# tuanad121/Python-WORLD

Measured on AMD Instinct MI355X. Metric: analysis+synthesis frames/sec (and xRT), 16 kHz / 5 ms hop, higher is better.
Workload: dtype f64; 1 GPU; BASELINE config 2 per GPU: 64 x 10 s synthetic 16 kHz utterances, DIO+StoneMask+CheapTrick+D4C encode + pulse-wise synthesis decode with on-device Philox noise (not the reference-parity host-noise path), HBM-resident; utterances_per_gpu=64, distinct_utterances=64, fs=16000, lanes_per_gpu=1

## Files before the change

### __graft_entry__.py

```python
import importlib.util
import os
import sys

ROOT = os.path.dirname(os.path.abspath(__file__))
PKG = os.path.join(ROOT, "python-world_amd")
for p in (ROOT, PKG):
    if p not in sys.path:
        sys.path.insert(0, p)


def build() -> None:
    spec = importlib.util.spec_from_file_location("_world_build", os.path.join(PKG, "build.py"))
    mod = importlib.util.module_from_spec(spec)
    spec.loader.exec_module(mod)
    lib = mod.build(force=False, verbose=True)
    assert os.path.exists(lib), lib
    from world import _hip

    handle = _hip.load_library()
    missing = [n for n in _hip.SIGNATURES if not hasattr(handle, n)]
    assert not missing, "missing C-ABI symbols: %s" % missing
    import oracle.api
    import subprocess

    from tests.test_hip_bounds import BOUNDS_TUS, VARIANT
    if not os.path.exists(VARIANT) or os.path.getmtime(VARIANT) < os.path.getmtime(lib):
        spec_arg = "bounds=" + ";".join("%s:-DWH_BOUNDS=1" % tu for tu in BOUNDS_TUS)
        r = subprocess.run([sys.executable, os.path.join(ROOT, "tools", "build_variants.py"), spec_arg], capture_output=True,
                           text=True)
        assert r.returncode == 0 and "bounds ok" in r.stdout, r.stdout[-2000:] + r.stderr[-2000:]
    from tests.test_hip_resample_bounds import VARIANT as RS_VARIANT, build_variant
    if not os.path.exists(RS_VARIANT) or os.path.getmtime(RS_VARIANT) < os.path.getmtime(lib):
        build_variant()
    from tests.test_hip_manifold_bounds import VARIANT as DS_VARIANT, build_variant as build_ds_variant
    if not os.path.exists(DS_VARIANT) or os.path.getmtime(DS_VARIANT) < os.path.getmtime(lib):
        build_ds_variant()
    from tests._fft_variant_script import VARIANT as NC_VARIANT, build_variant as build_nc_variant
    if not os.path.exists(NC_VARIANT) or os.path.getmtime(NC_VARIANT) < os.path.getmtime(lib):
        build_nc_variant()
    print("build ok:", lib, "ABI version", handle.wh_version(), "+ bounds variants")


def smoke() -> None:
    import numpy as np
    import torch

    assert torch.cuda.is_available(), "smoke() needs a GPU"
    from oracle import api as oapi
    from world._synthetic import synth_utterance
    from world.batch import WorldBatch

    fs = 16000
    xs = [synth_utterance(40, fs, 0.6), synth_utterance(41, fs, 0.5)]
    wb = WorldBatch(0)
    enc = wb.encode(xs, fs, f0_method="dio")
    rng = np.random.RandomState(0)
    noise = [rng.randn(2 * len(x)) for x in xs]
    y, y_off = wb.decode_device(enc, noise=noise)
    y = y.cpu().numpy()
    dicts = enc.to_dicts()
    for u, x in enumerate(xs):
        o = oapi.encode_np(fs, x, f0_method="dio")
        assert np.array_equal(dicts[u]["vuv"], o["vuv"])
        for key in ("f0", "spectrogram", "aperiodicity"):
            err = np.sqrt(np.mean((dicts[u][key] - o[key]) ** 2) / np.mean(o[key] ** 2))
            assert err < 1e-6, (key, err)
        yo = oapi.decode_np(dict(dicts[u]), noise=noise[u])["out"]
        seg = y[y_off[u]:y_off[u + 1]]
        assert len(seg) == len(yo)
        err = np.sqrt(np.mean((seg - yo) ** 2) / np.mean(yo ** 2))
        assert err < 1e-6, ("out", err)
    assert wb.rt.take_flags() == [0] * 16
    print("smoke ok: HIP encode+decode matches the oracle on %d utterances" % len(xs))


if __name__ == "__main__":
    build()
    if len(sys.argv) > 1 and sys.argv[1] == "smoke":
        smoke()
```

### python-world_amd/csrc/wh_synthesis.hip

```cpp
#include <type_traits>

#include "wh_host.h"
#include "wh_math.h"
__device__ __forceinline__ unsigned wh_opaque_tid() {
  unsigned t = threadIdx.x;
  asm volatile("" : "+v"(t));
  return t;
}
#define WH_TID wh_opaque_tid()
#include "wh_device.h"

#ifdef WH_RESP_STAGE_TIMER
__device__ unsigned long long g_resp_stage[16];
#define RSTAGE_BEGIN unsigned long long _t0 = __builtin_readcyclecounter();
#define RSTAGE_MARK(i) { __syncthreads(); if (threadIdx.x == 0) { const unsigned long long _t = __builtin_readcyclecounter(); atomicAdd(&g_resp_stage[i], _t - _t0); _t0 = _t; } }
#define RSTAGE_COUNT(i) { if (threadIdx.x == 0) atomicAdd(&g_resp_stage[i], 1ull); }
#else
#define RSTAGE_BEGIN
#define RSTAGE_MARK(i)
#define RSTAGE_COUNT(i)
#endif
namespace {

#ifndef WH_SYN_CONTRACT
#define WH_SYN_CONTRACT 0
#endif
#ifndef WH_RESP_TRANS_UNROLL
#define WH_RESP_TRANS_UNROLL 1
#endif
#ifndef WH_RESP_ABLATE
#define WH_RESP_ABLATE 0
#endif
#ifndef WH_RESP_ROLES
#define WH_RESP_ROLES 1
#endif
#ifndef WH_RESP_PAIR
#define WH_RESP_PAIR 1
#endif
#ifndef WH_RESP_SKIP_AP
#define WH_RESP_SKIP_AP 1
#endif
#ifndef WH_RESP_CONV8
#define WH_RESP_CONV8 1
#endif
#ifndef WH_FT_SYNTH
#define WH_FT_SYNTH 256
#endif
constexpr int ft_syn(int n) { return n >= 2048 ? 2 * WH_FT_SYNTH : WH_FT_SYNTH; }
template <int N>
constexpr bool resp_conv8() { return WH_RESP_CONV8 && N / ft_syn(N) == 4 && N >= 2048; }

struct SynUtt {
  int64_t f_off, nf;
  int64_t y_off, ny;
  int64_t p_off, pcap;
  int64_t noise_off, noise_len;
  double t0, dt;
};

__device__ __forceinline__ int64_t lerp_segment(const double* __restrict__ tp, int64_t nf, double t) {
  int64_t lo = 0, hi = nf;
  if (nf >= 2) {
    const double first = tp[0], last = tp[nf - 1];
    const double g = ceil((t - first) * (double)(nf - 1) / (last - first));
    if (g >= 1.0 && g <= (double)(nf - 1)) {
      const int64_t gi = (int64_t)g;
      const double a = tp[gi - 1], b = tp[gi], c = gi + 1 < nf ? tp[gi + 1] : b;
      if (a < t && !(b < t)) return gi;
      if (b < t && !(c < t) && gi + 1 <= nf - 1) return gi + 1;
      if (gi >= 2 && !(a < t) && tp[gi - 2] < t) return gi - 1;
    }
  }
  while (lo < hi) {
    const int64_t mid = (lo + hi) >> 1;
    if (tp[mid] < t) lo = mid + 1; else hi = mid;
  }
  return lo < 1 ? 1 : (lo > nf - 1 ? nf - 1 : lo);
}
__device__ __forceinline__ double lerp_on(const double* __restrict__ tp, const double* __restrict__ v, int64_t ih, double t) {
  const int64_t il = ih - 1;
  const double slope = (v[ih] - v[il]) / (tp[ih] - tp[il]);
  return slope * (t - tp[il]) + v[il];
}

__global__ __launch_bounds__(256) void prep_kernel(const SynUtt* __restrict__ meta, const double* __restrict__ tp,
                                                   const double* __restrict__ f0, const double* __restrict__ vuv,
                                                   double fs, double f0_low_limit, double* __restrict__ phase,
                                                   uint8_t* __restrict__ vuv_s) {
  const SynUtt m = meta[blockIdx.y];
  const int64_t i = (int64_t)blockIdx.x * 256 + threadIdx.x;
  if (i >= m.ny) return;
  const double t = m.t0 + (double)i * m.dt;
  const double* tpu = tp + m.f_off;
  const int64_t ih = lerp_segment(tpu, m.nf, t);
  double f_raw;
  if (f0_low_limit > 0.0) {
    const double* fu = f0 + m.f_off;
    const double* vu = vuv + m.f_off;
    auto final_f0 = [&](int64_t k) { return vu[k] == 0.0 ? 0.0 : (fu[k] < f0_low_limit ? 500.0 : fu[k]); };
    const int64_t il = ih - 1;
    const double slope = (final_f0(ih) - final_f0(il)) / (tpu[ih] - tpu[il]);
    f_raw = slope * (t - tpu[il]) + final_f0(il);
  } else {
    f_raw = lerp_on(tpu, f0 + m.f_off, ih, t);
  }
  const bool v = lerp_on(tpu, vuv + m.f_off, ih, t) > 0.5;
  double fi = f_raw * (v ? 1.0 : 0.0);
  if (fi == 0.0) fi = fi + 500.0;
  phase[m.y_off + i] = 2 * M_PI * fi / fs;
  vuv_s[m.y_off + i] = v ? 1 : 0;
}

#ifndef WH_XTILE
#define WH_XTILE 4096
#endif
constexpr int kXTile = WH_XTILE;
#ifndef WH_XTHREADS
#define WH_XTHREADS 512
#endif
constexpr int kXThreads = WH_XTHREADS;
// ... 604 lines not shown
  for (int r = 0; r < 10; ++r) {
    philox_round(c0, c1, c2, c3, k0, k1);
    k0 += 0x9E3779B9u;
    k1 += 0xBB67AE85u;
  }
  const double u1 = ((double)c0 * 4294967296.0 + (double)c1 + 0.5) * (1.0 / 18446744073709551616.0);
  const double u2 = ((double)c2 * 4294967296.0 + (double)c3 + 0.5) * (1.0 / 18446744073709551616.0);
  const double rr = sqrt(-2.0 * log(u1));
  double s, c;
  sincospi(2 * u2, &s, &c);
  return (q & 1) ? rr * s : rr * c;
}

__device__ __attribute__((noinline)) double2 normal_pair(uint64_t seed, uint64_t blk) {
  uint32_t c0 = (uint32_t)blk, c1 = (uint32_t)(blk >> 32), c2 = 0x9E3779B9u, c3 = 0x243F6A88u;
  uint32_t k0 = (uint32_t)seed, k1 = (uint32_t)(seed >> 32);
#pragma unroll
  for (int r = 0; r < 10; ++r) {
    philox_round(c0, c1, c2, c3, k0, k1);
    k0 += 0x9E3779B9u;
    k1 += 0xBB67AE85u;
  }
  const double u1 = ((double)c0 * 4294967296.0 + (double)c1 + 0.5) * (1.0 / 18446744073709551616.0);
  const double u2 = ((double)c2 * 4294967296.0 + (double)c3 + 0.5) * (1.0 / 18446744073709551616.0);
  const double rr = sqrt(-2.0 * log(u1));
  double s, c;
  sincospi(2 * u2, &s, &c);
  return make_double2(rr * c, rr * s);
}

__device__ __host__ __forceinline__ uint64_t philox_key(uint64_t seed, uint64_t u) {
  return seed * 0x9E3779B97F4A7C15ull + u * 0xD1B54A32D192ED03ull + 1;
}
__global__ __launch_bounds__(256) void philox_dump_kernel(uint64_t seed, int32_t u, int64_t q0, int64_t n,
                                                          double* __restrict__ out) {
  const int64_t i = (int64_t)blockIdx.x * 256 + threadIdx.x;
  if (i < n) out[i] = normal_at(philox_key(seed, (uint64_t)u), (uint64_t)(q0 + i));
}
__global__ __launch_bounds__(64) void noise_cover_kernel(const SynUtt* __restrict__ meta, const PulseRec* __restrict__ rec,
                                                         const int64_t* __restrict__ p_base, int n_utt,
                                                         int32_t* __restrict__ flags) {
  const int u = blockIdx.x * 64 + threadIdx.x;
  if (u >= n_utt) return;
  const int64_t count = p_base[u + 1] - p_base[u];
  if (count < 1) return;
  const PulseRec& r = rec[p_base[u] + count - 1];
  const int64_t need = r.noff + (r.noise_size > 3 ? r.noise_size : 3);
  if (meta[u].noise_len >= 0 && need > meta[u].noise_len) atomicOr(flags + WH_FLAG_NOISE_SHORT, 1);
}

#ifndef WH_FAST_MATH64
#define WH_FAST_MATH64 1
#endif
#ifndef WH_TRANS_PAIRS
#define WH_TRANS_PAIRS 1
#endif
__device__ __attribute__((noinline)) double4 cis_pair_call(double a0, double b0, double a1, double b1) {
  const double e0 = exp(a0), e1 = exp(a1);
  double s0, c0, s1, c1;
  sincospi(b0, &s0, &c0);
  sincospi(b1, &s1, &c1);
  return make_double4(e0 * c0, e0 * s0, e1 * c1, e1 * s1);
}
#if WH_FAST_MATH64
__device__ __attribute__((noinline)) double2 log_pair_call(double x, double y) { return make_double2(wh::flog(x), wh::flog(y)); }
__device__ __attribute__((noinline)) double log_call(double x) { return wh::flog(x); }
__device__ __attribute__((noinline)) double exp_call(double x) { return exp(x); }
__device__ __attribute__((noinline)) double2 sincospi_call(double x) {
  double s, c;
  sincospi(x, &s, &c);
  return make_double2(s, c);
}
#else
__device__ __attribute__((noinline)) double2 log_pair_call(double x, double y) { return make_double2(log(x), log(y)); }
__device__ __attribute__((noinline)) double log_call(double x) { return log(x); }
__device__ __attribute__((noinline)) double exp_call(double x) { return exp(x); }
__device__ __attribute__((noinline)) double2 sincospi_call(double x) {
  double s, c;
  sincospi(x, &s, &c);
  return make_double2(s, c);
}
#endif

template <int M, bool INV, int GT, int FT, bool WAVE>
__device__ __forceinline__ void mp_fft(wh::ckp<double2> zb, wh::ckp<const double2> tw) {
  if constexpr (WAVE) wh::fft_lds_wave<M, INV, GT, FT>(zb, tw);
  else wh::fft_lds<M, INV, GT, FT>(zb, tw);
}
template <int N>
constexpr bool resp_wave_fft() { return N == 1024; }
template <int N>
constexpr bool resp_skip_ap() { return WH_RESP_SKIP_AP && resp_wave_fft<N>(); }
struct SpectrumIdentity {
  __device__ __forceinline__ double2 operator()(int, double2 e) const { return e; }
};
struct NoSide {};
template <int N, int GT, bool WAVE = false, class Mul = SpectrumIdentity, class Side = NoSide>
__device__ __forceinline__ void min_phase_response(wh::ckp<double2> zb, wh::ckp<const double2> tw_base, double delay_pi, Mul mul = Mul(),
                                                   Side side = Side()) {
#if WH_SYN_CONTRACT
#pragma clang fp contract(fast)
#endif
  constexpr int FT = ft_syn(N);
  constexpr int M = N / 2;
  constexpr int PP = (M / 2 + 1 + GT - 1) / GT;
  const wh::ckp<double> zr = wh::ck_as<double>(zb);
  const int gt = WH_TID & (GT - 1);
  const wh::ckp<const double2> WH_RESTRICT w = tw_base + N;
#if defined(WH_RESP_ABLATE_T1) && WH_RESP_ABLATE_T1
  wh::sync<FT>();
#else
  if constexpr (WAVE && !std::is_same<Side, NoSide>::value) wh::fft_lds_wave<M, false, GT, FT>(zb, tw_base + M, side);
  else mp_fft<M, false, GT, FT, WAVE>(zb, tw_base + M);
#endif
  {
    double ck[PP], cm[PP];
#pragma unroll
    for (int p = 0; p < PP; ++p) {
      const int k = gt + p * GT;
      ck[p] = cm[p] = 0.0;
      if (k <= M / 2) {
        const double2 a = zb[k], b = zb[M - k];
        if (k == 0) {
          ck[p] = a.x + a.y;
          cm[p] = a.x - a.y;
        } else {
          const double er = 0.5 * (a.x + b.x), dr = 0.5 * (a.x - b.x), di = 0.5 * (a.y + b.y);
          const double2 wk = wh::ldg2(w + k);
          const double tr = fma(wk.x, di, wk.y * dr);
          ck[p] = er + tr;
          cm[p] = er - tr;
        }
      }
    }
    wh::sync<FT>();
#pragma unroll
    for (int p = 0; p < PP; ++p) {
      const int k = gt + p * GT;
      if (k <= M / 2) {
        if (k == 0) {
          zr[0] = ck[p];
          zr[M] = 2 * cm[p];
        } else {
          zr[N - k] = 2 * ck[p];
          zr[M + k] = 2 * cm[p];
        }
      }
    }
    for (int n = 1 + gt; n < M; n += GT) zr[n] = 0.0;
    wh::sync<FT>();
  }
  mp_fft<M, false, GT, FT, WAVE>(zb, tw_base + M);
#pragma unroll 1
  for (int k = gt; k <= M / 2; k += GT) {
    const double2 a = zb[k], b = zb[M - k];
    double2 x0, x1;
    const double2 wk = wh::ldg2(w + k);
    if (k == 0) {
      x0 = make_double2(a.x + a.y, 0.0);
      x1 = make_double2(a.x - a.y, 0.0);
    } else {
      const double er = 0.5 * (a.x + b.x), ei = 0.5 * (a.y - b.y);
      const double dr = 0.5 * (a.x - b.x), di = 0.5 * (a.y + b.y);
      const double tr = fma(wk.x, di, wk.y * dr);
      const double ti = fma(wk.y, di, -(wk.x * dr));
      x0 = make_double2(er + tr, ei + ti);
      x1 = make_double2(er - tr, ti - ei);
    }
#if WH_TRANS_PAIRS
    const double4 cis = cis_pair_call(x0.x / N, -x0.y / N * M_1_PI - delay_pi * (double)k, x1.x / N,
                                      -x1.y / N * M_1_PI - delay_pi * (double)(M - k));
    const double e0 = 1.0, e1 = 1.0;
    const double2 s0 = make_double2(cis.y, cis.x), s1 = make_double2(cis.w, cis.z);
#else
    const double e0 = exp_call(x0.x / N), e1 = exp_call(x1.x / N);
    const double2 s0 = sincospi_call(-x0.y / N * M_1_PI - delay_pi * (double)k);
    const double2 s1 = sincospi_call(-x1.y / N * M_1_PI - delay_pi * (double)(M - k));
#endif
    double2 A = mul(k, make_double2(e0 * s0.y, e0 * s0.x)), B = mul(M - k, make_double2(e1 * s1.y, e1 * s1.x));
    if (k == 0) {
      A.y = 0.0;
      B.y = 0.0;
    }
    const double er = A.x + B.x, ei = A.y - B.y;
    const double dr = A.x - B.x, di = A.y + B.y;
    const double orr = fma(dr, wk.x, di * wk.y);
    const double oi = fma(di, wk.x, -(dr * wk.y));
    zb[k] = make_double2(er - oi, ei + orr);
    if (k != 0) zb[M - k] = make_double2(er + oi, orr - ei);
  }
  wh::sync<FT>();
  mp_fft<M, true, GT, FT, WAVE>(zb, tw_base + M);
}

__device__ __forceinline__ int rap_index(int i) { return i + 2 * (i >> 5); }

__device__ __forceinline__ int first_pulse_at(const int64_t* __restrict__ pi, int count, int64_t lo) {
  const int lane = threadIdx.x & 63;
  int base = 0, n = count;
  while (n > 0) {
    const int stride = (n + 63) / 64;
    const int idx = base + lane * stride;
    const bool below = idx < base + n && pi[idx] < lo;
    const int c = __popcll(__ballot(below));
    if (stride == 1) {
      base += c;
      break;
    }
    if (c == 0) break;
    const int nb_ = base + (c - 1) * stride + 1;
    const int left = base + n - nb_;
    n = stride - 1 < left ? stride - 1 : left;
    base = nb_;
  }
  return base;
}

struct RespArgs {
  const SynUtt* meta;
  const double* tp;
  const double* spectrogram;
  const double* aperiodicity;
  double fs;
  const PulseRec* p_rec;
  const int64_t* p_base;
  int n_utt;
  const double* noise;
  uint64_t seed;
  const double* dc_base;
  const double2* tw_base;
  double* rows;
  const int64_t* row_base;
  const int64_t* run_base;
  const int64_t* row_off;
  int64_t runs_cap;
};

struct RunState {
  bool any;
  int64_t win_start;
  int64_t row_start;
  double last;
};
#ifndef WH_RESP_RUN
#define WH_RESP_RUN 0
#endif

template <int N>
__device__ __forceinline__ void ring_flush(wh::ckp<double> ring, int64_t a, int64_t b, wh::ckp<double> WH_RESTRICT row, int64_t row_start,
                                           int64_t ny) {
  constexpr int FT = ft_syn(N);
  a = a < 1 ? 1 : a;
  b = b > ny ? ny : b;
  for (int64_t tgt = a + WH_TID; tgt < b; tgt += FT) {
    const int slot = (int)(tgt & (N - 1));
    row[1 + (tgt - row_start)] = ring[slot];
    ring[slot] = 0.0;
  }
}

template <int R>
__device__ __forceinline__ void noise_conv_groups(wh::ckp<double> rap, wh::ckp<double> nzb, int cnt, int m0, int64_t j0, double (&acc)[R]) {
#if WH_SYN_CONTRACT
#pragma clang fp contract(fast)
#endif
  auto load_group = [&](int base, double (&g)[R]) {
#pragma unroll
    for (int t = 0; t < R; t += 2) {
      double2 v = make_double2(0.0, 0.0);
      if (base >= 0) v = wh::ck_as<const double2>(rap + rap_index(base + t))[0];
      g[t] = v.x;
      g[t + 1] = v.y;
    }
  };
  auto block = [&](int j, const double (&hi)[R], const double (&lo)[R]) {
    double n[R];
#pragma unroll
    for (int t = 0; t < R; t += 2) {
      const double2 v = wh::ck_as<const double2>(nzb + (j + t))[0];
      n[t] = v.x;
      n[t + 1] = v.y;
    }
#pragma unroll
    for (int sft = 0; sft < R; ++sft)
#pragma unroll
      for (int q = 0; q < R; ++q) acc[q] = fma(n[sft], q - sft >= 0 ? hi[q - sft] : lo[R + q - sft], acc[q]);
  };
  double ga[R], gb[R];
  const int mb0 = m0 - (int)j0;
  load_group(mb0, ga);
  load_group(mb0 - R, gb);
  const int steps = ((cnt + 2 * R - 1) / (2 * R)) * (2 * R);
  for (int j = 0; j < steps; j += 2 * R) {
    block(j, ga, gb);
    load_group(mb0 - j - 2 * R, ga);
    block(j + R, gb, ga);
    load_group(mb0 - j - 3 * R, gb);
  }
}

template <int N>
__device__ __forceinline__ void ring_advance(wh::ckp<double> ring, RunState& rs, wh::ckp<double> WH_RESTRICT row, int64_t s1, int64_t ny) {
  constexpr int FT = ft_syn(N);
  if (rs.any) {
    const int64_t e = s1 < rs.win_start + N ? s1 : rs.win_start + N;
    ring_flush<N>(ring, rs.win_start, e, row, rs.row_start, ny);
    for (int64_t tgt = rs.win_start + N + WH_TID; tgt < (s1 < ny ? s1 : ny); tgt += FT) row[1 + (tgt - rs.row_start)] = 0.0;
    wh::sync<FT>();
  } else {
    rs.row_start = s1 < 1 ? 1 : s1;
  }
  rs.any = true;
  rs.win_start = s1;
}

template <int N>
__device__ __forceinline__ void response_pulse(const RespArgs& A, const PulseRec& rec, char* smem, wh::ckp<double> ring, RunState& rs,
                                               wh::ckp<double> WH_RESTRICT row,
                                               const double (&dcw)[N / ft_syn(N) <= 4 ? N / ft_syn(N) : 1]) {
#if WH_SYN_CONTRACT
#pragma clang fp contract(fast)
#endif
  const SynUtt* __restrict__ meta = A.meta;
  const double* __restrict__ spectrogram = A.spectrogram;
  const double* __restrict__ aperiodicity = A.aperiodicity;
  const double fs = A.fs;
  const double* __restrict__ noise = A.noise;
  const uint64_t seed = A.seed;
  const double* __restrict__ dc_base = A.dc_base;
  const double2* __restrict__ tw_raw = A.tw_base;
  asm volatile("" : "+s"(tw_raw));
  const wh::ckp<const double2> tw_base = wh::ck_make(tw_raw, WH_TWIDDLE_ENTRIES, wh::WH_CK_TWIDDLE);
  constexpr int FT = ft_syn(N);
  constexpr int K = N / 2 + 1;
  constexpr int NZ = 256;
  constexpr int NZC = resp_conv8<N>() ? 252 : NZ;
  constexpr int R = N / FT;
  static_assert(R % 2 == 0 && NZ % (2 * R) == 0, "pairwise reads; whole blocks of 2R noise samples");
  constexpr int GT = FT >= 256 ? FT / 2 : FT;
  constexpr int NG = FT / GT;
  const wh::ckp<double> lds_all = wh::ck_make(reinterpret_cast<double*>(smem), 2 * (N + 2) + (N + N / 16 + 2) + NZ + 32, wh::WH_CK_LDS_OTHER);
  const wh::ckp<double> zrA = wh::ck_sub(lds_all, 0, N + 2, wh::WH_CK_LDS_MAIN);
  const wh::ckp<double2> zbA = wh::ck_as<double2>(zrA);
  const wh::ckp<double> zrP = wh::ck_sub(lds_all, N + 2, N + 2, wh::WH_CK_LDS_AUX);
  const wh::ckp<double2> zbP = wh::ck_as<double2>(zrP);
  const wh::ckp<double> rap = wh::ck_sub(lds_all, 2 * (N + 2), N + N / 16 + 2, wh::WH_CK_LDS_OTHER);
  const wh::ckp<double> nz = wh::ck_sub(lds_all, 2 * (N + 2) + (N + N / 16 + 2), NZ, wh::WH_CK_LDS_OTHER);
  const wh::ckp<double> scratch = wh::ck_sub(lds_all, 2 * (N + 2) + (N + N / 16 + 2) + NZ, 32, wh::WH_CK_LDS_SCRATCH);

  RSTAGE_BEGIN
  wh::sync<FT>();
  const int u = rec.u;
  const SynUtt m = meta[u];
  const int64_t pidx = rec.pidx;
  const double shift = rec.shift;
  const int64_t noise_size = rec.noise_size;

  const int64_t row_lo = rec.rows & 0xffffffffll, row_hi = rec.rows >> 32;
  const double bw = rec.weight;
  const bool same = bw < 0.0;
  const double b = same ? 0.0 : bw;
  const double a = 1 - b;
  const double* s_lo = spectrogram + row_lo * K;
  const double* s_hi = spectrogram + row_hi * K;
  const double* a_lo = aperiodicity + row_lo * K;
  const double* a_hi = aperiodicity + row_hi * K;
  constexpr int KQ = (K + FT - 1) / FT;
  double rsl[KQ], rsh[KQ], ral[KQ], rah[KQ];
  const bool need_ap = rec.vuv != 0;
#pragma unroll
  for (int q = 0; q < KQ; ++q) {
    const int k = WH_TID + q * FT;
    const int kc = k < K ? k : K - 1;
    rsl[q] = s_lo[kc];
    rsh[q] = s_hi[kc];
    if constexpr (resp_skip_ap<N>()) {
      ral[q] = rah[q] = 0.0;
    } else {
      ral[q] = a_lo[kc];
      rah[q] = a_hi[kc];
    }
  }
  double ap0_lo, ap0_hi;
  if constexpr (resp_skip_ap<N>()) {
    ap0_lo = ap0_hi = 0.0;
    if (need_ap) {
#pragma unroll
      for (int q = 0; q < KQ; ++q) {
        const int k = WH_TID + q * FT;
        const int kc = k < K ? k : K - 1;
        ral[q] = a_lo[kc];
        rah[q] = a_hi[kc];
      }
      ap0_lo = a_lo[0];
      ap0_hi = a_hi[0];
    }
  } else {
    ap0_lo = a_lo[0];
    ap0_hi = a_hi[0];
  }
  asm volatile("" : "+v"(ap0_lo), "+v"(ap0_hi));
  double aper0;
  {
    const double al = ap0_lo * ap0_lo, ah = ap0_hi * ap0_hi;
    aper0 = same ? al : a * al + b * ah;
  }
  const bool voiced = (rec.vuv != 0) && (aper0 <= 0.999);
  RSTAGE_COUNT(voiced ? 8 : (rec.vuv == 0 ? 9 : 10))
  RSTAGE_COUNT(13)
#pragma unroll
  for (int q = 0; q < KQ; ++q) {
    const int k = WH_TID + q * FT;
    if (k >= K) break;
    const double sl = rsl[q], sh = rsh[q];
    double v, w;
    auto spectra = [&]() {
      double al = ral[q] * ral[q], ah = rah[q] * rah[q];
      if constexpr (resp_skip_ap<N>()) asm volatile("" : "+v"(al), "+v"(ah));
      const double pl = fmax(0.001, 1 - al), ph = fmax(0.001, 1 - ah);
      const double sp = same ? sl : a * sl + b * sh;
      const double pe = same ? pl : a * pl + b * ph;
      const double ap = same ? al : a * al + b * ah;
      v = sp * pe;
      if (v == 0.0) v = 2.220446049250313e-16;
      w = voiced ? sp * ap : sp;
    };
    if constexpr (resp_skip_ap<N>()) {
      v = 0.0;
      w = same ? sl : a * sl + b * sh;
      if (voiced) spectra();
    } else {
      spectra();
    }
    if (w == 0.0) w = 2.220446049250313e-16;
#if WH_TRANS_PAIRS
    double2 lg;
    if (voiced) lg = log_pair_call(fabs(w), fabs(v));
    else lg = make_double2(log_call(fabs(w)), 0.0);
    const double lw = lg.x / 2;
#else
    const double lw = log_call(fabs(w)) / 2;
#endif
    zrA[k] = lw;
    if (k > 0 && k < N / 2) zrA[N - k] = lw;
    if (voiced) {
#if WH_TRANS_PAIRS
      const double lv = lg.y / 2;
#else
      const double lv = log_call(fabs(v)) / 2;
#endif
      zrP[k] = lv;
      if (k > 0 && k < N / 2) zrP[N - k] = lv;
    }
  }
  RSTAGE_MARK(5)
  const int64_t nd = noise_size > 3 ? noise_size : 3;
  const int64_t noff = rec.noff;
  auto noise_at = [&](int64_t j) -> double {
    if (noise) {
      const int64_t q = noff + j;
      return q < m.noise_len ? noise[m.noise_off + q] : 0.0;
    }
    return normal_at(philox_key(seed, (uint64_t)u), (uint64_t)(noff + j));
  };
  constexpr bool ROLES = WH_RESP_ROLES && resp_wave_fft<N>();
  static_assert(!ROLES || NZ / 2 + 1 <= FT, "a run that fits nz is at most one Philox block per thread");
  const bool side_noise = ROLES && noise == nullptr && nd <= NZ;
  auto noise_side = [&](int i, int n) {
    if (!side_noise) return;
    const uint64_t key = philox_key(seed, (uint64_t)u);
    const int lane = i & 63;
    const int64_t blk0 = noff >> 1, b1 = (noff + nd - 1) >> 1;
    for (int c = __builtin_amdgcn_readfirstlane(i - lane); blk0 + c <= b1; c += n) {
      const int64_t blk = blk0 + c + lane;
      double part = 0.0;
      if (blk <= b1) {
        const double2 z = normal_pair(key, (uint64_t)blk);
        const int64_t j = 2 * blk - noff;
        if (j >= 0) {
          part += z.x;
          nz[j] = z.x;
        }
        if (j + 1 < nd) {
          part += z.y;
          nz[j + 1] = z.y;
        }
      }
      part = wh::wave_sum(part);
      if (lane == 0) scratch[c >> 6] = part;
    }
  };
  double mean = 0.0;
  if (side_noise) {
    wh::sync<FT>();
  } else {
    double part = 0.0;
    if (noise) {
      for (int64_t j = WH_TID; j < nd; j += FT) {
        const double v = noise_at(j);
        part += v;
        if (j < NZ) nz[j] = v;
      }
    } else {
      const uint64_t key = philox_key(seed, (uint64_t)u);
      const int64_t b1 = (noff + nd - 1) >> 1;
      for (int64_t blk = (noff >> 1) + WH_TID; blk <= b1; blk += FT) {
        const double2 z = normal_pair(key, (uint64_t)blk);
        const int64_t j = 2 * blk - noff;
        if (j >= 0) {
          part += z.x;
          if (j < NZ) nz[j] = z.x;
        }
        if (j + 1 < nd) {
          part += z.y;
          if (j + 1 < NZ) nz[j + 1] = z.y;
        }
      }
    }
    mean = wh::block_sum<FT>(part, scratch) / (double)nd;
  }

  RSTAGE_MARK(0)
#if WH_RESP_ABLATE == 2
  if (WH_TID == 0) row[0] = zrA[3] + zrP[5] + mean;
  return;
#endif
  const double coef_pi = 2.0 * fs / N;
  if constexpr (ROLES) {
    if (NG == 2 && voiced) {
      const int g = WH_TID / GT;
      min_phase_response<N, GT, true>(g == 0 ? zbA : zbP, tw_base, g == 0 ? 0.0 : coef_pi * shift, SpectrumIdentity(), noise_side);
    } else {
      min_phase_response<N, FT, true>(zbA, tw_base, 0.0, SpectrumIdentity(), noise_side);
      if (voiced) min_phase_response<N, FT, true>(zbP, tw_base, coef_pi * shift);
    }
  } else if (NG == 2 && voiced) {
    const int g = WH_TID / GT;
    min_phase_response<N, GT, resp_wave_fft<N>()>(g == 0 ? zbA : zbP, tw_base, g == 0 ? 0.0 : coef_pi * shift);
  } else {
    min_phase_response<N, FT, resp_wave_fft<N>()>(zbA, tw_base, 0.0);
    if (voiced) min_phase_response<N, FT, resp_wave_fft<N>()>(zbP, tw_base, coef_pi * shift);
  }
  RSTAGE_MARK(voiced ? 2 : 6)
  if (side_noise) {
    const int n_blk = (int)(((noff + nd - 1) >> 1) - (noff >> 1)) + 1;
    double t = 0.0;
#pragma unroll
    for (int w = 0; w < (NZ / 2 + 1 + 63) / 64; ++w)
      if (w * 64 < n_blk) t += scratch[w];
    mean = t / (double)nd;
  }
  for (int n = WH_TID; n < N; n += FT) rap[rap_index(n)] = zrA[(n + N / 2) & (N - 1)] / N;
  wh::sync<FT>();

  double acc[R];
#pragma unroll
  for (int q = 0; q < R; ++q) acc[q] = 0.0;
  double acc8[resp_conv8<N>() ? 8 : 1];
#pragma unroll
  for (int q = 0; q < (resp_conv8<N>() ? 8 : 1); ++q) acc8[q] = 0.0;
  const int m0 = WH_TID * R;
#if WH_RESP_ABLATE == 1
  for (int64_t j0 = 0; j0 < 0; j0 += NZC) {
#else
  for (int64_t j0 = 0; j0 < nd; j0 += NZC) {
#endif
    const int cnt = (int)(nd - j0 < NZC ? nd - j0 : NZC);
    wh::sync<FT>();
    for (int j = WH_TID; j < NZ; j += FT) {
      double v = 0.0;
      if (j < cnt) v = (j0 == 0 ? nz[j] : noise_at(j0 + j)) - mean;
      nz[j] = v;
    }
    wh::sync<FT>();
    if constexpr (resp_conv8<N>()) {
      constexpr int HT = FT / 2;
      const int half_id = WH_TID / HT, t8 = WH_TID - half_id * HT;
      const int c_all = ((cnt + 11) / 12) * 12;
      const int c_mid = ((c_all / 12 + 1) / 2) * 12;
      const int jb = half_id == 0 ? 0 : c_mid, je = half_id == 0 ? c_mid : c_all;
      auto load4 = [&](int base, double (&g)[4]) {
        double2 v0 = make_double2(0.0, 0.0), v1 = make_double2(0.0, 0.0);
        if (base >= 0) {
          v0 = wh::ck_as<const double2>(rap + rap_index(base))[0];
          v1 = wh::ck_as<const double2>(rap + rap_index(base + 2))[0];
        }
        g[0] = v0.x; g[1] = v0.y; g[2] = v1.x; g[3] = v1.y;
      };
      auto block4 = [&](int j, const double (&hi)[4], const double (&mid)[4], const double (&lo)[4]) {
#pragma unroll
        for (int sp = 0; sp < 4; sp += 2) {
          const double2 nn = wh::ck_as<const double2>(nz + (j + sp))[0];
#pragma unroll
          for (int sft = sp; sft < sp + 2; ++sft)
#pragma unroll
            for (int q = 0; q < 8; ++q) {
              const int idx = q - sft;
              acc8[q] = fma(sft == sp ? nn.x : nn.y, idx >= 4 ? hi[idx - 4] : (idx >= 0 ? mid[idx] : lo[idx + 4]), acc8[q]);
            }
        }
      };
      const int mb0 = t8 * 8 - (int)j0 - jb;
      double g0[4], g1[4], g2[4];
      load4(mb0 + 4, g0);
      load4(mb0, g1);
      load4(mb0 - 4, g2);
      for (int j = jb; j < je; j += 12) {
        const int mb = t8 * 8 - (int)j0 - j;
        block4(j, g0, g1, g2);
        load4(mb - 8, g0);
        block4(j + 4, g1, g2, g0);
        load4(mb - 12, g1);
        block4(j + 8, g2, g0, g1);
        load4(mb - 16, g2);
      }
    } else if constexpr (R <= 4) {
      auto load_group = [&](int base, double (&g)[R]) {
  #pragma unroll
        for (int t = 0; t < R; t += 2) {
          double2 v = make_double2(0.0, 0.0);
          if (base >= 0) v = wh::ck_as<const double2>(rap + rap_index(base + t))[0];
          g[t] = v.x;
          g[t + 1] = v.y;
        }
      };
      auto block = [&](int j, const double (&hi)[R], const double (&lo)[R]) {
        double n[R];
  #pragma unroll
        for (int t = 0; t < R; t += 2) {
          const double2 v = wh::ck_as<const double2>(nz + (j + t))[0];
          n[t] = v.x;
          n[t + 1] = v.y;
        }
  #pragma unroll
        for (int sft = 0; sft < R; ++sft)
  #pragma unroll
// ... 280 lines not shown
    if (r < n_runs) {
      const int kf = r * RUN;
      const int kl = (kf + RUN < count ? kf + RUN : count) - 1;
      int64_t start = pi[kf] - N / 2 + 1, end = pi[kl] + N / 2 + 1;
      start = start < 1 ? 1 : start;
      end = end < m.ny ? end : m.ny;
      len = 1 + (int)(end > start ? end - start : 0);
    }
    int total;
    const int excl = block_excl_scan_256(len, wsum, &total);
    if (r < n_runs) {
      const int64_t at = carry + excl;
      const bool fits = at + len <= room;
      out[r] = fits ? at : -1;
      over = over || !fits;
    }
    carry += total;
    __syncthreads();
  }
  if (over) atomicOr(flags + WH_FLAG_PULSE_OVERFLOW, 1);
}

template <int N>
__global__ __launch_bounds__(ft_syn(N), 4) void response_kernel(RespArgs A) {
  extern __shared__ __attribute__((aligned(16))) char smem[];
  constexpr int FT = ft_syn(N);
  constexpr int RUN = resp_run(N);
  const int64_t n_runs = A.run_base[A.n_utt];
  const int64_t run = wh::xcd_unit(blockIdx.x, n_runs);
  if (run >= n_runs) return;
  int u = 0;
  {
    int lo = 0, hi = A.n_utt;
    while (hi - lo > 1) {
      const int mid = (lo + hi) >> 1;
      if (A.run_base[mid] <= run) lo = mid; else hi = mid;
    }
    u = lo;
  }
  const int64_t r_in_utt = run - A.run_base[u];
  const wh::ckp<double> ring = wh::ck_make(reinterpret_cast<double*>(smem) + (2 * (N + 2) + (N + N / 16 + 2) + 256 + 32), N, wh::WH_CK_LDS_OTHER);
  for (int i = threadIdx.x; i < N; i += FT) ring[i] = 0.0;
  RunState rs{false, 0, 1, 0.0};
  const int64_t gp0 = A.p_base[u] + r_in_utt * RUN;
  const int64_t gp1 = gp0 + RUN < A.p_base[u + 1] ? gp0 + RUN : A.p_base[u + 1];
  const int64_t my_off = A.row_off[(int64_t)u * A.runs_cap + r_in_utt];
  if (my_off < 0) return;
  const wh::ckp<double> row = wh::ck_make(A.rows + A.row_base[u] + my_off, A.row_base[u + 1] - A.row_base[u] - my_off, wh::WH_CK_OUT);
  auto fetch_rec = [&](int64_t gp) -> uint32_t {
    return reinterpret_cast<const uint32_t*>(A.p_rec + gp)[threadIdx.x & 15];
  };
  auto unpack_rec = [&](uint32_t word) -> PulseRec {
    uint32_t d[16];
#pragma unroll
    for (int i = 0; i < 13; ++i) d[i] = (uint32_t)__builtin_amdgcn_readlane((int)word, i);
    PulseRec r;
    r.pidx = (int64_t)(((uint64_t)d[1] << 32) | d[0]);
    r.rows = (int64_t)(((uint64_t)d[3] << 32) | d[2]);
    r.weight = __hiloint2double((int)d[5], (int)d[4]);
    r.shift = __hiloint2double((int)d[7], (int)d[6]);
    r.noff = (int64_t)(((uint64_t)d[9] << 32) | d[8]);
    r.u = (int32_t)d[10];
    r.noise_size = (int32_t)d[11];
    r.vuv = (int32_t)d[12];
    r.pad_[0] = r.pad_[1] = r.pad_[2] = 0;
    return r;
  };
  uint32_t cur_w = fetch_rec(gp0);
  constexpr int R = N / FT;
  double dcw[R <= 4 ? R : 1];
  if constexpr (R <= 4) {
#pragma unroll
    for (int q = 0; q < R; ++q) dcw[q] = A.dc_base[threadIdx.x * R + q];
  } else {
    dcw[0] = 0.0;
  }
  int64_t row_start;
  {
    const int64_t pidx0 = reinterpret_cast<const int64_t*>(A.p_rec + gp0)[0];
    row_start = pidx0 - N / 2 + 1;
    row_start = row_start < 1 ? 1 : row_start;
  }
  (void)row_start;
  if constexpr (resp_pairs<N>()) {
    uint32_t nxt_w = fetch_rec(gp0 + 1 < gp1 ? gp0 + 1 : gp0);
#pragma unroll 1
    for (int64_t gp = gp0; gp < gp1;) {
      const PulseRec cur = unpack_rec(cur_w);
      const int64_t last = gp1 - 1;
      bool pair = false;
      if (gp + 1 < gp1)
        pair = resp_pairable(A, cur.vuv, cur.noise_size, __builtin_amdgcn_readlane((int)nxt_w, 12), __builtin_amdgcn_readlane((int)nxt_w, 11));
      if (pair) {
        const PulseRec nxt = unpack_rec(nxt_w);
        const uint32_t w2 = fetch_rec(gp + 2 < last ? gp + 2 : last), w3 = fetch_rec(gp + 3 < last ? gp + 3 : last);
        response_pair<N>(A, cur, nxt, smem, ring, rs, row);
        cur_w = w2;
        nxt_w = w3;
        gp += 2;
      } else {
        const uint32_t w2 = fetch_rec(gp + 2 < last ? gp + 2 : last);
        response_pulse<N>(A, cur, smem, ring, rs, row, dcw);
        cur_w = nxt_w;
        nxt_w = w2;
        gp += 1;
      }
    }
  } else {
#pragma unroll 1
    for (int64_t gp = gp0; gp < gp1; ++gp) {
      const PulseRec cur = unpack_rec(cur_w);
      const uint32_t nxt_w = fetch_rec(gp + 1 < gp1 ? gp + 1 : gp);
#ifdef WH_RESP_STAGE_TIMER
      if (gp + 1 < gp1 && resp_pairable(A, cur.vuv, cur.noise_size, __builtin_amdgcn_readlane((int)nxt_w, 12), __builtin_amdgcn_readlane((int)nxt_w, 11)))
        RSTAGE_COUNT(11)
#endif
      response_pulse<N>(A, cur, smem, ring, rs, row, dcw);
      cur_w = nxt_w;
    }
  }
  wh::sync<FT>();
  if (rs.any) ring_flush<N>(ring, rs.win_start, rs.win_start + N, row, rs.row_start, A.meta[u].ny);
  if (threadIdx.x == FT - 1) row[0] = rs.last;
}

#ifndef WH_GATHER_PER
#define WH_GATHER_PER 4
#endif
constexpr int kGatherTile = 256 * WH_GATHER_PER;
template <int N>
__global__ __launch_bounds__(256) void response_gather_kernel(const SynUtt* __restrict__ meta,
                                                              const int64_t* __restrict__ p_idx,
                                                              const int32_t* __restrict__ p_count,
                                                              const double* __restrict__ rows, const int64_t* __restrict__ row_base,
                                                              const int64_t* __restrict__ row_off, int64_t runs_cap,
                                                              double* __restrict__ y) {
  constexpr int RUN = resp_run(N);
  constexpr int PER = WH_GATHER_PER;
  const SynUtt m = meta[blockIdx.y];
  const int64_t n0 = (int64_t)blockIdx.x * kGatherTile;
  if (n0 >= m.ny) return;
  const int count = p_count[blockIdx.y];
  const int64_t* pi = p_idx + m.p_off;
  const double* ru = rows + row_base[blockIdx.y];
  const int64_t* ro = row_off + (int64_t)blockIdx.y * runs_cap;
  const int k0 = first_pulse_at(pi, count, n0 + 1 - N / 2);
  const int n_runs = (count + RUN - 1) / RUN;
  double sum[PER];
#pragma unroll
  for (int q = 0; q < PER; ++q) sum[q] = 0.0;
  const int64_t t0 = n0 + 1 + threadIdx.x;
  for (int r = k0 / RUN; r < n_runs; ++r) {
    const int kf = r * RUN;
    const int kl = (kf + RUN < count ? kf + RUN : count) - 1;
    const int64_t s1f = pi[kf] - N / 2 + 1;
    if (s1f > n0 + kGatherTile) break;
    const int64_t start = s1f < 1 ? 1 : s1f;
    int64_t end = pi[kl] + N / 2 + 1;
    end = end < m.ny ? end : m.ny;
    const int64_t off = ro[r];
    if (off < 0) continue;
    const double* rr = ru + off + 1 - start;
#pragma unroll
    for (int q = 0; q < PER; ++q) {
      const int64_t tgt = t0 + 256 * q;
      if (tgt >= start && tgt < end) sum[q] += rr[tgt];
    }
  }
#pragma unroll
  for (int q = 0; q < PER; ++q) {
    const int64_t tgt = t0 + 256 * q;
    if (tgt < m.ny) y[m.y_off + tgt - 1] = sum[q];
  }
  if (n0 + kGatherTile >= m.ny) {
    const int k_end = first_pulse_at(pi, count, m.ny - N / 2);
    if (threadIdx.x == 0) {
      double last = 0.0;
      for (int r = k_end / RUN; r < n_runs; ++r) {
        const int64_t off = ro[r];
        if (off >= 0) last += ru[off];
      }
      y[m.y_off + m.ny - 1] = last;
    }
  }
}


template <int N>
int launch_resp(wh_ctx* ctx, hipStream_t st, int B, int64_t pcap_max, int64_t max_ny, const std::vector<int64_t>& h_ny, const SynUtt* d_meta, const double* tp,
                const double* spec, const double* ap, double fs, const PulseRec* p_rec, const int64_t* p_base,
                const int64_t* p_idx, const int32_t* p_count, const double* noise, uint64_t seed, double* y) {
  std::vector<double> dc(N);
  double sum = 0.0;
  for (int n = 0; n < N; ++n) {
    dc[n] = 0.5 - 0.5 * cos(2.0 * M_PI * (double)(n + 1) / (double)(N + 1));
    sum += dc[n];
  }
  for (int n = 0; n < N; ++n) dc[n] /= sum;
  const double* d_dc = nullptr;
  if (int rc = wh::const_table(ctx, "dc_base:" + std::to_string(N), dc, &d_dc)) return rc;
  const size_t lds = sizeof(double) * (2 * (N + 2) + (N + N / 16 + 2) + 256 + 32 + N);
  if (int rc = wh::allow_lds(&response_kernel<N>, lds)) return rc;
  const int64_t runs_cap = (pcap_max + resp_run(N) - 1) / resp_run(N);
  int64_t per_sample = (96 * pcap_max + max_ny - 1) / (max_ny > 0 ? max_ny : 1);
  per_sample = per_sample < 12 ? 12 : (per_sample > 48 ? 48 : per_sample);
  std::vector<int64_t> row_base((size_t)B + 1, 0);
// ... 705 lines not shown
```

Baseline: 14.73 million frames/s.

## Prefetch next voiced pulse's log spectra during current pulse's FFT side slots

```diff
diff --git a/__graft_entry__.py b/__graft_entry__.py
--- a/__graft_entry__.py
+++ b/__graft_entry__.py
@@ -38,6 +38,9 @@
     from tests._fft_variant_script import VARIANT as NC_VARIANT, build_variant as build_nc_variant
     if not os.path.exists(NC_VARIANT) or os.path.getmtime(NC_VARIANT) < os.path.getmtime(lib):
         build_nc_variant()
+    from tests._prefetch_variant_script import VARIANT as NP_VARIANT, build_variant as build_np_variant
+    if not os.path.exists(NP_VARIANT) or os.path.getmtime(NP_VARIANT) < os.path.getmtime(lib):
+        build_np_variant()
     print("build ok:", lib, "ABI version", handle.wh_version(), "+ bounds variants")
 
 
diff --git a/python-world_amd/csrc/wh_synthesis.hip b/python-world_amd/csrc/wh_synthesis.hip
--- a/python-world_amd/csrc/wh_synthesis.hip
+++ b/python-world_amd/csrc/wh_synthesis.hip
@@ -36,6 +36,9 @@
 #endif
 #ifndef WH_RESP_PAIR
 #define WH_RESP_PAIR 1
+#endif
+#ifndef WH_RESP_PREFETCH
+#define WH_RESP_PREFETCH 1
 #endif
 #ifndef WH_RESP_SKIP_AP
 #define WH_RESP_SKIP_AP 1
@@ -806,22 +809,28 @@
 }
 #endif
 
-template <int M, bool INV, int GT, int FT, bool WAVE>
-__device__ __forceinline__ void mp_fft(wh::ckp<double2> zb, wh::ckp<const double2> tw) {
-  if constexpr (WAVE) wh::fft_lds_wave<M, INV, GT, FT>(zb, tw);
-  else wh::fft_lds<M, INV, GT, FT>(zb, tw);
+struct NoSide {};
+template <int M, bool INV, int GT, int FT, bool WAVE, class Side = NoSide>
+__device__ __forceinline__ void mp_fft(wh::ckp<double2> zb, wh::ckp<const double2> tw, Side side = Side()) {
+  if constexpr (WAVE) {
+    if constexpr (std::is_same<Side, NoSide>::value) wh::fft_lds_wave<M, INV, GT, FT>(zb, tw);
+    else wh::fft_lds_wave<M, INV, GT, FT>(zb, tw, side);
+  } else {
+    wh::fft_lds<M, INV, GT, FT>(zb, tw);
+  }
 }
 template <int N>
 constexpr bool resp_wave_fft() { return N == 1024; }
 template <int N>
 constexpr bool resp_skip_ap() { return WH_RESP_SKIP_AP && resp_wave_fft<N>(); }
+template <int N>
+constexpr bool resp_prefetch() { return WH_RESP_PREFETCH && WH_RESP_PAIR && WH_RESP_ROLES && resp_wave_fft<N>() && ft_syn(N) == 256; }
 struct SpectrumIdentity {
   __device__ __forceinline__ double2 operator()(int, double2 e) const { return e; }
 };
-struct NoSide {};
-template <int N, int GT, bool WAVE = false, class Mul = SpectrumIdentity, class Side = NoSide>
+template <int N, int GT, bool WAVE = false, class Mul = SpectrumIdentity, class Side = NoSide, class Side2 = NoSide, class Side3 = NoSide>
 __device__ __forceinline__ void min_phase_response(wh::ckp<double2> zb, wh::ckp<const double2> tw_base, double delay_pi, Mul mul = Mul(),
-                                                   Side side = Side()) {
+                                                   Side side = Side(), Side2 side2 = Side2(), Side3 side3 = Side3()) {
 #if WH_SYN_CONTRACT
 #pragma clang fp contract(fast)
 #endif
@@ -834,8 +843,7 @@
 #if defined(WH_RESP_ABLATE_T1) && WH_RESP_ABLATE_T1
   wh::sync<FT>();
 #else
-  if constexpr (WAVE && !std::is_same<Side, NoSide>::value) wh::fft_lds_wave<M, false, GT, FT>(zb, tw_base + M, side);
-  else mp_fft<M, false, GT, FT, WAVE>(zb, tw_base + M);
+  mp_fft<M, false, GT, FT, WAVE>(zb, tw_base + M, side);
 #endif
   {
     double ck[PP], cm[PP];
@@ -874,7 +882,7 @@
     for (int n = 1 + gt; n < M; n += GT) zr[n] = 0.0;
     wh::sync<FT>();
   }
-  mp_fft<M, false, GT, FT, WAVE>(zb, tw_base + M);
+  mp_fft<M, false, GT, FT, WAVE>(zb, tw_base + M, side2);
 #pragma unroll 1
   for (int k = gt; k <= M / 2; k += GT) {
     const double2 a = zb[k], b = zb[M - k];
@@ -914,7 +922,7 @@
     if (k != 0) zb[M - k] = make_double2(er + oi, orr - ei);
   }
   wh::sync<FT>();
-  mp_fft<M, true, GT, FT, WAVE>(zb, tw_base + M);
+  mp_fft<M, true, GT, FT, WAVE>(zb, tw_base + M, side3);
 }
 
 __device__ __forceinline__ int rap_index(int i) { return i + 2 * (i >> 5); }
@@ -1041,7 +1049,12 @@
 template <int N>
 __device__ __forceinline__ void response_pulse(const RespArgs& A, const PulseRec& rec, char* smem, wh::ckp<double> ring, RunState& rs,
                                                wh::ckp<double> WH_RESTRICT row,
-                                               const double (&dcw)[N / ft_syn(N) <= 4 ? N / ft_syn(N) : 1]) {
+                                               const double (&dcw)[N / ft_syn(N) <= 4 ? N / ft_syn(N) : 1], uint32_t nxt_w, bool nxt_ok,
+                                               bool& parked
+#ifdef WH_RESP_STAGE_TIMER
+                                               , bool& t_prev
+#endif
+                                               ) {
 #if WH_SYN_CONTRACT
 #pragma clang fp contract(fast)
 #endif
@@ -1092,30 +1105,38 @@
   constexpr int KQ = (K + FT - 1) / FT;
   double rsl[KQ], rsh[KQ], ral[KQ], rah[KQ];
   const bool need_ap = rec.vuv != 0;
-#pragma unroll
-  for (int q = 0; q < KQ; ++q) {
-    const int k = WH_TID + q * FT;
-    const int kc = k < K ? k : K - 1;
-    rsl[q] = s_lo[kc];
-    rsh[q] = s_hi[kc];
-    if constexpr (resp_skip_ap<N>()) {
-      ral[q] = rah[q] = 0.0;
-    } else {
+  bool pre = false;
+  if constexpr (resp_prefetch<N>()) pre = parked;
+  auto load_rows = [&]() {
+#pragma unroll
+    for (int q = 0; q < KQ; ++q) {
+      const int k = WH_TID + q * FT;
+      const int kc = k < K ? k : K - 1;
+      rsl[q] = s_lo[kc];
+      rsh[q] = s_hi[kc];
+      if constexpr (resp_skip_ap<N>()) {
+        ral[q] = rah[q] = 0.0;
+      } else {
+        ral[q] = a_lo[kc];
+        rah[q] = a_hi[kc];
+      }
+    }
+  };
+  auto load_ap_rows = [&]() {
+#pragma unroll
+    for (int q = 0; q < KQ; ++q) {
+      const int k = WH_TID + q * FT;
+      const int kc = k < K ? k : K - 1;
       ral[q] = a_lo[kc];
       rah[q] = a_hi[kc];
     }
-  }
+  };
+  if (!pre) load_rows();
   double ap0_lo, ap0_hi;
   if constexpr (resp_skip_ap<N>()) {
     ap0_lo = ap0_hi = 0.0;
     if (need_ap) {
-#pragma unroll
-      for (int q = 0; q < KQ; ++q) {
-        const int k = WH_TID + q * FT;
-        const int kc = k < K ? k : K - 1;
-        ral[q] = a_lo[kc];
-        rah[q] = a_hi[kc];
-      }
+      if (!pre) load_ap_rows();
       ap0_lo = a_lo[0];
       ap0_hi = a_hi[0];
     }
@@ -1132,26 +1153,56 @@
   const bool voiced = (rec.vuv != 0) && (aper0 <= 0.999);
   RSTAGE_COUNT(voiced ? 8 : (rec.vuv == 0 ? 9 : 10))
   RSTAGE_COUNT(13)
+  const bool expanded = pre && voiced;
+  if (expanded) {
+    static_assert(!resp_prefetch<N>() || (KQ == 3 && K == 2 * FT + 1), "two bins per thread and the Nyquist bin");
+    double pk[2], am[2], pn = 0.0;
+#pragma unroll
+    for (int q = 0; q < 2; ++q) {
+      const int k = WH_TID + q * FT;
+      pk[q] = zrA[K + k];
+      am[q] = zrA[k];
+    }
+    if (WH_TID == 0) pn = zrA[K + N / 2];
+    wh::sync<FT>();
+#pragma unroll
+    for (int q = 0; q < 2; ++q) {
+      const int k = WH_TID + q * FT;
+      zrP[k] = pk[q];
+      if (k > 0) {
+        zrA[N - k] = am[q];
+        zrP[N - k] = pk[q];
+      }
+    }
+    if (WH_TID == 0) zrP[N / 2] = pn;
+  } else if (pre) {
+    load_rows();
+    load_ap_rows();
+  }
 #pragma unroll
   for (int q = 0; q < KQ; ++q) {
     const int k = WH_TID + q * FT;
-    if (k >= K) break;
+    if (k >= K || expanded) break;
     const double sl = rsl[q], sh = rsh[q];
     double v, w;
+    auto mix = [&](double x, double y) -> double {
+      if constexpr (resp_prefetch<N>()) return fma(a, x, b * y);
+      else return a * x + b * y;
+    };
     auto spectra = [&]() {
       double al = ral[q] * ral[q], ah = rah[q] * rah[q];
       if constexpr (resp_skip_ap<N>()) asm volatile("" : "+v"(al), "+v"(ah));
       const double pl = fmax(0.001, 1 - al), ph = fmax(0.001, 1 - ah);
-      const double sp = same ? sl : a * sl + b * sh;
-      const double pe = same ? pl : a * pl + b * ph;
-      const double ap = same ? al : a * al + b * ah;
+      const double sp = same ? sl : mix(sl, sh);
+      const double pe = same ? pl : mix(pl, ph);
+      const double ap = same ? al : mix(al, ah);
       v = sp * pe;
       if (v == 0.0) v = 2.220446049250313e-16;
       w = voiced ? sp * ap : sp;
     };
     if constexpr (resp_skip_ap<N>()) {
       v = 0.0;
-      w = same ? sl : a * sl + b * sh;
+      w = same ? sl : mix(sl, sh);
       if (voiced) spectra();
     } else {
       spectra();
@@ -1177,7 +1228,14 @@
       if (k > 0 && k < N / 2) zrP[N - k] = lv;
     }
   }
-  RSTAGE_MARK(5)
+#ifdef WH_RESP_STAGE_TIMER
+  {
+    const bool single_voiced = WH_RESP_ROLES && resp_wave_fft<N>() && voiced && noise == nullptr && (rec.noise_size > 3 ? rec.noise_size : 3) <= 256;
+    if (single_voiced && t_prev) RSTAGE_COUNT(15)
+    t_prev = single_voiced;
+    RSTAGE_MARK(single_voiced ? 14 : 5)
+  }
+#endif
   const int64_t nd = noise_size > 3 ? noise_size : 3;
   const int64_t noff = rec.noff;
   auto noise_at = [&](int64_t j) -> double {
@@ -1214,6 +1272,58 @@
       if (lane == 0) scratch[c >> 6] = part;
     }
   };
+  constexpr bool PF = resp_prefetch<N>();
+  static_assert(!PF || 2 * K - N <= 2, "the values beyond N go to the first pair of padding slots");
+  auto park_slot = [](int j) { return j < N ? rap_index(j) : 32 + (j - N); };
+  const bool produce = PF && nxt_ok && voiced && side_noise;
+  auto log_side = [&](int i, auto k_first, auto k_end) {
+    constexpr int K0 = decltype(k_first)::value, K1 = decltype(k_end)::value, ST = FT - NG * WH_WAVE;
+    constexpr int SQ = (K1 - K0 + ST - 1) / ST;
+    const int64_t rows1 = (int64_t)(((uint64_t)(uint32_t)__builtin_amdgcn_readlane((int)nxt_w, 3) << 32) | (uint32_t)__builtin_amdgcn_readlane((int)nxt_w, 2));
+    const double bw1 = __hiloint2double(__builtin_amdgcn_readlane((int)nxt_w, 5), __builtin_amdgcn_readlane((int)nxt_w, 4));
+    const bool same1 = bw1 < 0.0;
+    const double b1 = same1 ? 0.0 : bw1;
+    const double a1 = 1 - b1;
+    const int64_t lo1 = rows1 & 0xffffffffll, hi1 = rows1 >> 32;
+    const double* s_lo1 = spectrogram + lo1 * K;
+    const double* s_hi1 = spectrogram + hi1 * K;
+    const double* a_lo1 = aperiodicity + lo1 * K;
+    const double* a_hi1 = aperiodicity + hi1 * K;
+    double sl[SQ], sh[SQ], rl[SQ], rh[SQ];
+#pragma unroll
+    for (int q = 0; q < SQ; ++q) {
+      const int k = K0 + i + q * ST;
+      const int kc = k < K1 ? k : K1 - 1;
+      sl[q] = s_lo1[kc];
+      sh[q] = s_hi1[kc];
+      rl[q] = a_lo1[kc];
+      rh[q] = a_hi1[kc];
+    }
+#pragma unroll
+    for (int q = 0; q < SQ; ++q) {
+      const int k = K0 + i + q * ST;
+      if (k >= K1) break;
+      double al = rl[q] * rl[q], ah = rh[q] * rh[q];
+      asm volatile("" : "+v"(al), "+v"(ah));
+      const double pl = fmax(0.001, 1 - al), ph = fmax(0.001, 1 - ah);
+      const double sp = same1 ? sl[q] : fma(a1, sl[q], b1 * sh[q]);
+      const double pe = same1 ? pl : fma(a1, pl, b1 * ph);
+      const double ap = same1 ? al : fma(a1, al, b1 * ah);
+      double v = sp * pe;
+      if (v == 0.0) v = 2.220446049250313e-16;
+      double w = sp * ap;
+      if (w == 0.0) w = 2.220446049250313e-16;
+      const double2 lg = log_pair_call(fabs(w), fabs(v));
+      rap[park_slot(k)] = lg.x / 2;
+      rap[park_slot(K + k)] = lg.y / 2;
+    }
+  };
+  auto log_side2 = [&](int i, int) {
+    if (produce) log_side(i, std::integral_constant<int, 0>(), std::integral_constant<int, N / 4>());
+  };
+  auto log_side3 = [&](int i, int) {
+    if (produce) log_side(i, std::integral_constant<int, N / 4>(), std::integral_constant<int, K>());
+  };
   double mean = 0.0;
   if (side_noise) {
     wh::sync<FT>();
@@ -1253,7 +1363,11 @@
   if constexpr (ROLES) {
     if (NG == 2 && voiced) {
       const int g = WH_TID / GT;
-      min_phase_response<N, GT, true>(g == 0 ? zbA : zbP, tw_base, g == 0 ? 0.0 : coef_pi * shift, SpectrumIdentity(), noise_side);
+      if constexpr (PF)
+        min_phase_response<N, GT, true>(g == 0 ? zbA : zbP, tw_base, g == 0 ? 0.0 : coef_pi * shift, SpectrumIdentity(), noise_side, log_side2,
+                                        log_side3);
+      else
+        min_phase_response<N, GT, true>(g == 0 ? zbA : zbP, tw_base, g == 0 ? 0.0 : coef_pi * shift, SpectrumIdentity(), noise_side);
     } else {
       min_phase_response<N, FT, true>(zbA, tw_base, 0.0, SpectrumIdentity(), noise_side);
       if (voiced) min_phase_response<N, FT, true>(zbP, tw_base, coef_pi * shift);
@@ -1274,8 +1388,29 @@
       if (w * 64 < n_blk) t += scratch[w];
     mean = t / (double)nd;
   }
+  constexpr int PKQ = PF ? (2 * K + FT - 1) / FT : 1;
+  [[maybe_unused]] double park[PKQ];
+  if constexpr (PF) {
+    if (produce) {
+#pragma unroll
+      for (int q = 0; q < PKQ; ++q) {
+        const int j = WH_TID + q * FT;
+        park[q] = j < 2 * K ? rap[park_slot(j)] : 0.0;
+      }
+    }
+  }
   for (int n = WH_TID; n < N; n += FT) rap[rap_index(n)] = zrA[(n + N / 2) & (N - 1)] / N;
   wh::sync<FT>();
+  if constexpr (PF) {
+    if (produce) {
+#pragma unroll
+      for (int q = 0; q < PKQ; ++q) {
+        const int j = WH_TID + q * FT;
+        if (j < 2 * K) zrA[j] = park[q];
+      }
+    }
+    parked = produce;
+  }
 
   double acc[R];
 #pragma unroll
@@ -1722,6 +1857,13 @@
     row_start = row_start < 1 ? 1 : row_start;
   }
   (void)row_start;
+  bool parked = false;
+#ifdef WH_RESP_STAGE_TIMER
+  bool t_prev = false;
+#define RSTAGE_ARG , t_prev
+#else
+#define RSTAGE_ARG
+#endif
   if constexpr (resp_pairs<N>()) {
     uint32_t nxt_w = fetch_rec(gp0 + 1 < gp1 ? gp0 + 1 : gp0);
 #pragma unroll 1
@@ -1735,12 +1877,19 @@
         const PulseRec nxt = unpack_rec(nxt_w);
         const uint32_t w2 = fetch_rec(gp + 2 < last ? gp + 2 : last), w3 = fetch_rec(gp + 3 < last ? gp + 3 : last);
         response_pair<N>(A, cur, nxt, smem, ring, rs, row);
+#ifdef WH_RESP_STAGE_TIMER
+        t_prev = false;
+#endif
         cur_w = w2;
         nxt_w = w3;
         gp += 2;
       } else {
         const uint32_t w2 = fetch_rec(gp + 2 < last ? gp + 2 : last);
-        response_pulse<N>(A, cur, smem, ring, rs, row, dcw);
+        bool nxt_ok = false;
+        if constexpr (resp_prefetch<N>())
+          nxt_ok = gp + 1 < gp1 && A.noise == nullptr && __builtin_amdgcn_readlane((int)nxt_w, 12) != 0 &&
+                   __builtin_amdgcn_readlane((int)nxt_w, 11) <= 256;
+        response_pulse<N>(A, cur, smem, ring, rs, row, dcw, nxt_w, nxt_ok, parked RSTAGE_ARG);
         cur_w = nxt_w;
         nxt_w = w2;
         gp += 1;
@@ -1755,13 +1904,14 @@
       if (gp + 1 < gp1 && resp_pairable(A, cur.vuv, cur.noise_size, __builtin_amdgcn_readlane((int)nxt_w, 12), __builtin_amdgcn_readlane((int)nxt_w, 11)))
         RSTAGE_COUNT(11)
 #endif
-      response_pulse<N>(A, cur, smem, ring, rs, row, dcw);
+      response_pulse<N>(A, cur, smem, ring, rs, row, dcw, nxt_w, false, parked RSTAGE_ARG);
       cur_w = nxt_w;
     }
   }
   wh::sync<FT>();
   if (rs.any) ring_flush<N>(ring, rs.win_start, rs.win_start + N, row, rs.row_start, A.meta[u].ny);
   if (threadIdx.x == FT - 1) row[0] = rs.last;
+#undef RSTAGE_ARG
 }
 
 #ifndef WH_GATHER_PER
```

After: 14.77 million frames/s, median of 6. About the same (+0.2%).
